# may-/joeys2t

Hardware: AMD Instinct MI355X
Metric: audio frames/sec (train step, 80-mel, 15 s utt, bs32 per GPU) (higher is better)
Workload: dtype bf16; 1 GPU; configs/librispeech_100h.yaml ASR train step on synthetic 16 kHz waveforms; global_batch=32, frames_per_utt=1498, encoder_len=375, lengths=fixed 15 s, vocab=5000, batch_multiplier=1, parallelism=dp1, launch=hipGraph replay

## Files before the change

### include/joeys2t_hip.h

```cpp
#ifndef JOEYS2T_HIP_H
#define JOEYS2T_HIP_H

#include <stdint.h>

#ifdef __cplusplus
extern "C" {
#endif

typedef void* js2t_stream;

enum { JS2T_F32 = 0, JS2T_BF16 = 1, JS2T_FP8_E4M3 = 2  };
enum { JS2T_ACT_NONE = 0, JS2T_ACT_RELU = 1, JS2T_ACT_GELU = 2, JS2T_ACT_SWISH = 3, JS2T_ACT_TANH = 4, JS2T_ACT_HARDSWISH = 5 };
enum { JS2T_OK = 0, JS2T_ERR_INVALID = -1, JS2T_ERR_LAUNCH = -2, JS2T_ERR_UNSUPPORTED = -3 };

int js2t_abi_version(void);
const char* js2t_last_error(void);

typedef struct js2t_gemm_desc {
  int32_t M, N, K;
  int32_t batch, batch_inner;
  int32_t dtype_ab, dtype_c;
  int32_t trans_a, trans_b;
  const void* A; int64_t lda, a_stride_o, a_stride_i;
  const void* B; int64_t ldb, b_stride_o, b_stride_i;
// ... 26 lines not shown
  float* c8_state;
  const float* c8_mul;
  float* c8_scale_out;
  float* fp8_state;
  const void* dot_src;
  int64_t ld_dot;
  float* dot_partial;
  float* sumsq_partial;
} js2t_gemm_desc;

int js2t_gemm(const js2t_gemm_desc* d, js2t_stream stream);
#define JS2T_GEMM_GROUP_MAX 32
int js2t_gemm_grouped(const js2t_gemm_desc* d, int32_t count, const void* const* A, const void* const* B, void* const* C,
                      float* const* a_rowsum, js2t_stream stream);
int64_t js2t_gemm_grouped_blocks(int32_t M, int32_t N, int32_t count);
void js2t_gemm_force_regstage(int on);
void js2t_gemm_force_w256(int on);
void js2t_gemm_p192_mode(int mode);
void js2t_gemm_wg256_mode(int mode);
void js2t_gemm_p192_ring(int nst);
void js2t_gemm_panel_mode(int mode);


int js2t_axpby(const void* x, float a, const void* y, float b, void* out, int64_t n, int dt, js2t_stream stream);

int js2t_cast(const void* src, int src_dt, void* dst, int dst_dt, int64_t n, js2t_stream stream);

int js2t_fold_ln_weights(const int64_t* table, int32_t n_entries, int32_t max_rows, js2t_stream stream);

int js2t_absmax(const void* x, int dt, int64_t n, float* out, js2t_stream stream);
// ... 261 lines not shown
```

### joeys2t_amd/_lib.py

```python
import ctypes as C
import os
import re
from pathlib import Path

PKG_DIR = Path(__file__).resolve().parent
LIB_PATH = Path(os.environ.get("JS2T_LIB", PKG_DIR / "libjoeys2t_hip.so"))
HEADER_PATH = PKG_DIR.parent / "include" / "joeys2t_hip.h"

F32, BF16 = 0, 1
ACT_CODES = {None: 0, "none": 0, "relu": 1, "gelu": 2, "swish": 3, "tanh": 4, "hardswish": 5}


class Js2tError(RuntimeError):
    pass


_CTYPES = {
    "int": C.c_int, "int32_t": C.c_int32, "uint32_t": C.c_uint32, "int64_t": C.c_int64, "uint64_t": C.c_uint64,
    "float": C.c_float, "double": C.c_double, "js2t_stream": C.c_void_p, "js2t_ctx": C.c_void_p,
}


def _ctype(spelling: str, decl: str, ret: bool = False):
    t = " ".join(spelling.replace("*", " * ").split())
# ... 28 lines not shown
        raise Js2tError(f"{HEADER_PATH.name}: could not parse the declaration of {sorted(missed)}")
    return structs, functions


if not HEADER_PATH.exists():
    raise Js2tError(f"{HEADER_PATH} is missing: the Python binding reads every struct and signature from it")
STRUCTS, FUNCTIONS = parse_header(HEADER_PATH.read_text())


class GemmDesc(C.Structure):
    _fields_ = STRUCTS["js2t_gemm_desc"]


class AttnDesc(C.Structure):
    _fields_ = STRUCTS["js2t_attn_desc"]


def declared_symbols():
    return sorted(FUNCTIONS)


_lib = None


def lib():
    global _lib
    if _lib is None:
        if not LIB_PATH.exists():
            raise Js2tError(
                f"{LIB_PATH} is missing: the HIP extension has not been built "
# ... 66 lines not shown
```

### joeys2t_amd/csrc/gemm.hip

```cpp
#include "gemm_shared.hpp"
#include <type_traits>

namespace {

bool g_force_regstage = false;
bool g_force_w256 = false;

__device__ __forceinline__ bool a_elem_offset(const js2t_gemm_desc& d, int slow, int fast, int64_t& off) {
  if (!d.conv) {
    off = (int64_t)slow * d.lda + fast;
    return true;
  }
  const int b = slow / d.conv_tout, t = slow - b * d.conv_tout;
  const int kw = fast / d.conv_c;
  const int tin = t * d.conv_stride - d.conv_pad + kw;
  off = ((int64_t)b * d.conv_tin + (t * d.conv_stride - d.conv_pad)) * d.conv_c + fast;
  return tin >= 0 && tin < d.conv_tin;
}

__device__ __forceinline__ void gemm_epilogue4(const js2t_gemm_desc& d, int z, int64_t c_boff, int m, int n,
                                               f32x4_t acc, float alpha) {
  if (m >= d.M || n >= d.N) return;
  const int nv = min(4, d.N - n);
  float v[4];
// ... 2223 lines not shown
          const int m = tm0 + 16 * (w + 4 * i) + 4 * g + e;
          if (m < M) __builtin_amdgcn_global_atomic_fadd_f32((gfloat*)grp.rowsum[mem] + m, racc[i][e]);
        }
    }
  }
  P192_T(6);
  asm volatile("s_waitcnt vmcnt(0)" ::: "memory");
#ifdef JS2T_P192_PROF
  if (blockIdx.x == 0 && t == 0)
    for (int i = 0; i < 8; ++i) g_p192_prof[i] = prof_[i];
#endif
}

constexpr int WG_IMG = 16384, WG_STAGE = 3 * WG_IMG, WG_NST = 3, WG_LDS = WG_NST * WG_STAGE, WG_PER = 12;

template <bool RS, bool SPLITK>
__global__ __launch_bounds__(768, 1) void gemm_bf16_wg256_kernel(js2t_gemm_desc d, GemmGroup grp, int tiles_m, int tiles_n, int split_k) {
  extern __shared__ __attribute__((aligned(16))) unsigned char smem[];
  const int t = threadIdx.x, lane = t & 63;
  const int w = __builtin_amdgcn_readfirstlane(t >> 6);
  const int tiles = tiles_m * tiles_n;
  const int lid = xcd_remap(blockIdx.x, gridDim.x);
  const int vm = lid / tiles, tile = lid - vm * tiles;
  const int mem = SPLITK ? vm / split_k : vm, slice = SPLITK ? vm - mem * split_k : 0;
  const int m0 = (tile / tiles_n) * 256, n0 = (tile % tiles_n) * 128;
  const int K = d.K, nk_all = (K + 63) >> 6;
  const int per = SPLITK ? (nk_all + split_k - 1) / split_k : nk_all;
  const int kt0 = slice * per;
  const int nk = min(per, nk_all - kt0);
  float ss = 0.f;

  if (w >= 8) {
    const int l = w - 8;
    const int64_t lda = d.lda, ldb = d.ldb;
    const uint16_t* zsrc = (const uint16_t*)&g_zero16;
    const uint16_t* src[12];
    int krow[4];
    {
      const uint16_t* Ab = (const uint16_t*)grp.A[mem];
      const uint16_t* Bb = (const uint16_t*)grp.B[mem];
#pragma unroll
      for (int q = 0; q < 4; ++q) {
        const int p = (l * 4 + q) * 64 + lane, kr = p >> 4, col = (((p & 15) ^ (tr_g(kr) << 1)) << 3);
        krow[q] = kr;
        src[q] = Ab + (int64_t)kr * lda + m0 + col;
        src[4 + q] = Ab + (int64_t)kr * lda + m0 + 128 + col;
        src[8 + q] = Bb + (int64_t)kr * ldb + n0 + col;
      }
    }
    auto issue_stage = [&](int st, int slot) {
      const int k0 = st < nk ? (kt0 + st) << 6 : 0;
      const int64_t ka = (int64_t)k0 * lda, kb = (int64_t)k0 * ldb;
      const int klim = K - k0;
      unsigned char* stp = smem + slot * WG_STAGE + l * 4096;
#pragma unroll
      for (int q = 0; q < 12; ++q) {
        const uint16_t* sp = src[q] + (q < 8 ? ka : kb);
        if (klim < 64) {
          if (krow[q & 3] >= klim) sp = zsrc;
        }
        lds_dma16(sp, stp + (q >> 2) * WG_IMG + (q & 3) * 1024);
      }
    };
    issue_stage(0, 0);
    issue_stage(1, 1);
    asm volatile("s_waitcnt vmcnt(%0)" ::"n"(WG_PER) : "memory");
    __builtin_amdgcn_s_barrier();
    asm volatile("" ::: "memory");
    issue_stage(2, 2);
    int cslot = 0;
#ifdef JS2T_P192_PROF
    unsigned long long prof_[8] = {0, 0, 0, 0, 0, 0, 0, 0}, last_ = __builtin_readcyclecounter();
#endif
    for (int s = 0; s < nk; ++s) {
// ... 10 lines not shown
#ifdef JS2T_P192_PROF
    if (blockIdx.x == 0 && t == 512)
      for (int i = 4; i < 8; ++i) g_p192_prof[i] = prof_[i];
#endif
  } else {
    const int wm = w >> 1, wn = w & 1;
    const int a_img = (wm >> 1) * WG_IMG, a_sub = (wm & 1) * 64, b_sub = wn * 64;
    bf16x8_t fm0[4], fn0[4], fm1[4], fn1[4];
    f32x4_t acc[4][4], racc[4];
#pragma unroll
    for (int i = 0; i < 4; ++i) {
      racc[i] = f32x4_t{0.f, 0.f, 0.f, 0.f};
#pragma unroll
      for (int j = 0; j < 4; ++j) acc[i][j] = f32x4_t{0.f, 0.f, 0.f, 0.f};
    }
    const bool do_rs = RS && n0 == 0 && wn == 0 && grp.rowsum[mem] != nullptr;
    typedef __attribute__((ext_vector_type(8))) short s16x8_ones_t;
    const bf16x8_t ones = __builtin_bit_cast(bf16x8_t, s16x8_ones_t{0x3f80, 0x3f80, 0x3f80, 0x3f80, 0x3f80, 0x3f80, 0x3f80, 0x3f80});

    __builtin_amdgcn_s_barrier();
    asm volatile("" ::: "memory");
#pragma unroll
    for (int i = 0; i < 4; ++i) {
      fm0[i] = frag_load2<true>(smem + a_img, a_sub + 16 * i, 0, lane);
      fn0[i] = frag_load2<true>(smem + 2 * WG_IMG, b_sub + 16 * i, 0, lane);
    }
    int cslot = 0;
#ifdef JS2T_P192_PROF
    unsigned long long prof_[8] = {0, 0, 0, 0, 0, 0, 0, 0}, last_ = __builtin_readcyclecounter();
#endif
    for (int s = 0; s < nk; ++s) {
// ... 43 lines not shown
        for (int i = 0; i < 4; ++i) racc[i] = __builtin_amdgcn_mfma_f32_16x16x32_bf16(ones, fm1[i], racc[i], 0, 0, 0);
      }
      __builtin_amdgcn_sched_barrier(0);
      P192_T(3);
      cslot = nslot;
    }
#ifdef JS2T_P192_PROF
    if (blockIdx.x == 0 && t == 0)
      for (int i = 0; i < 4; ++i) g_p192_prof[i] = prof_[i];
#endif

    if (RS && do_rs && (lane >> 4) == 0) {
      typedef __attribute__((address_space(1))) float gfloat;
#pragma unroll
      for (int i = 0; i < 4; ++i)
        __builtin_amdgcn_global_atomic_fadd_f32((gfloat*)grp.rowsum[mem] + m0 + wm * 64 + 16 * i + lane, racc[i][0]);
    }
    if constexpr (SPLITK) {
      asm volatile("s_waitcnt lgkmcnt(0)" ::: "memory");
      __syncthreads();
      float* Cs = (float*)smem;
#pragma unroll
      for (int i = 0; i < 4; ++i)
#pragma unroll
        for (int j = 0; j < 4; ++j) {
          const int ml = wm * 64 + 16 * i + (lane & 15), n4 = wn * 16 + 4 * j + (lane >> 4);
          *(f32x4_t*)(Cs + ml * 128 + ((n4 ^ (ml & 7)) << 2)) = acc[i][j];
        }
    } else {
    const float alpha = d.alpha * (d.alpha_dev ? *d.alpha_dev : 1.f), beta = d.beta;
    float* Cb = (float*)grp.C[mem] + (int64_t)(m0 + wm * 64 + (lane & 15)) * d.ldc + n0 + wn * 64 + 4 * (lane >> 4);
#pragma unroll
    for (int i = 0; i < 4; ++i) {
      float* crow = Cb + (int64_t)(16 * i) * d.ldc;
      float4 old[4];
      if (beta != 0.f) {
#pragma unroll
        for (int j = 0; j < 4; ++j) old[j] = *(const float4*)(crow + 16 * j);
      }
#pragma unroll
      for (int j = 0; j < 4; ++j) {
        float4 v = make_float4(acc[i][j][0] * alpha, acc[i][j][1] * alpha, acc[i][j][2] * alpha, acc[i][j][3] * alpha);
        if (beta != 0.f) v.x += beta * old[j].x, v.y += beta * old[j].y, v.z += beta * old[j].z, v.w += beta * old[j].w;
        *(float4*)(crow + 16 * j) = v;
        ss = fmaf(v.x, v.x, fmaf(v.y, v.y, fmaf(v.z, v.z, fmaf(v.w, v.w, ss))));
      }
    }
    }
  }
  if constexpr (SPLITK) {
    if (w >= 8) __syncthreads();
    __syncthreads();
    const float alpha = d.alpha * (d.alpha_dev ? *d.alpha_dev : 1.f);
    const float* Cs = (const float*)smem;
    typedef __attribute__((address_space(1))) float gfloat;
    gfloat* cg = (gfloat*)grp.C[mem] + (int64_t)m0 * d.ldc + n0;
    for (int idx = w; idx < 512; idx += 12) {
      const int ml = idx >> 1, nl = (idx & 1) * 64 + lane;
      const float v = Cs[ml * 128 + ((((nl >> 2) ^ (ml & 7)) << 2) | (nl & 3))];
      __builtin_amdgcn_global_atomic_fadd_f32(cg + (int64_t)ml * d.ldc + nl, v * alpha);
    }
    return;
  }
  if (d.sumsq_partial) {
    ss = block_sum(ss, (float*)smem);
    if (t == 0) d.sumsq_partial[2 * blockIdx.x] = ss, d.sumsq_partial[2 * blockIdx.x + 1] = 0.f;
  }
}

#define g_p192_mode js2t_ctx_value(JS2T_CTX_GEMM_P192_MODE)
inline bool p192_eligible(const js2t_gemm_desc& d) {
  if (g_p192_mode == 0) return false;
  if (d.trans_a || d.trans_b || d.conv || d.split_k > 1 || d.batch != 1 || d.dtype_c != JS2T_BF16) return false;
  if ((d.N & 7) || d.N < 128 || (d.K & 7) || d.K < 192 || d.M < 1) return false;
  if (d.preact || d.beta != 0.f || !(d.act == JS2T_ACT_NONE || d.act == JS2T_ACT_RELU) || (d.residual && d.gate)) return false;
  if (!epilogue_rows_aligned(d)) return false;
  if (g_p192_mode < 0 && (int64_t)cdiv(d.M, P_BM) * (d.N >> 7) < 200) return false;
  return true;
}
#define g_p192_ring js2t_ctx_value(JS2T_CTX_GEMM_P192_RING)
enum P192Form { P192_LOADER_CONSUMER, P192_RING2, P192_RING3 };
inline P192Form p192_form(int tiles, int n_cu, int ring, bool stats_dot, bool fp8, bool c8, bool scaled) {
// ... 202 lines not shown
      else
        rc = a_rowsum ? launch_grouped_wg256<true, false>(d, grp, n, (hipStream_t)stream) : launch_grouped_wg256<false, false>(d, grp, n, (hipStream_t)stream);
    } else if (!d.sumsq_partial && p192t_eligible(d, n)) {
      rc = a_rowsum ? launch_grouped_p192t<true>(d, grp, n, (hipStream_t)stream) : launch_grouped_p192t<false>(d, grp, n, (hipStream_t)stream);
    } else {
      rc = d.split_k > 1 ? launch_grouped_tt<true>(d, grp, n, (hipStream_t)stream) : launch_grouped_tt<false>(d, grp, n, (hipStream_t)stream);
    }
    if (rc != JS2T_OK) return rc;
    if (d.sumsq_partial) d.sumsq_partial += (int64_t)cdiv(d.M, 128) * cdiv(d.N, F_BN) * n;
  }
  return JS2T_OK;
}

extern "C" int64_t js2t_gemm_grouped_blocks(int32_t M, int32_t N, int32_t count) {
  return (int64_t)cdiv(M, 128) * cdiv(N, F_BN) * count;
}

extern "C" int js2t_gemm(const js2t_gemm_desc* dp, js2t_stream stream) {
  JS2T_CHECK(dp != nullptr, "gemm: null descriptor");
  js2t_gemm_desc d = *dp;
  JS2T_CHECK(!d.sumsq_partial, "gemm: sumsq_partial is taken by js2t_gemm_grouped only");
  hipStream_t s = (hipStream_t)stream;
  JS2T_CHECK(d.M >= 0 && d.N >= 0 && d.K >= 0 && d.batch >= 0, "gemm: negative size");
  if (d.M == 0 || d.N == 0 || d.batch == 0) return JS2T_OK;
  JS2T_CHECK(d.A && d.B && (d.C || (d.c8 && d.dtype_ab == JS2T_FP8_E4M3)), "gemm: null operand");
  JS2T_CHECK(!d.c8 || (d.dtype_ab == JS2T_FP8_E4M3 && d.c8_state && d.ldc8 >= d.N && (d.ldc8 & 7) == 0 && aligned(d.c8, 8) &&
                       aligned(d.c8_state)),
             "gemm: c8 (e4m3 second output) needs e4m3 operands, c8_state (16-byte aligned) and 8-byte aligned rows");
  JS2T_CHECK(d.batch_inner >= 1, "gemm: batch_inner must be >= 1");
  JS2T_CHECK(d.dtype_ab == JS2T_F32 || d.dtype_ab == JS2T_BF16 || d.dtype_ab == JS2T_FP8_E4M3, "gemm: bad dtype_ab");
// ... 71 lines not shown
```

### joeys2t_amd/ops.py

```python
import ctypes as C
import math
from typing import Optional, Sequence

import torch

from joeys2t_amd._lib import ACT_CODES, BF16, F32, AttnDesc, GemmDesc, Js2tError, check, lib

FP8 = 2
_DT = {torch.float32: F32, torch.bfloat16: BF16, torch.float8_e4m3fn: FP8}


def dt_code(t_or_dtype) -> int:
    dtype = t_or_dtype.dtype if torch.is_tensor(t_or_dtype) else t_or_dtype
    try:
        return _DT[dtype]
    except KeyError:
        raise Js2tError(f"unsupported dtype {dtype}: the HIP path computes in float32 or bfloat16") from None


def _dev(*tensors):
    for t in tensors:
        if t is not None and not t.is_cuda:
            raise Js2tError(
                "joeys2t_amd ops run on the GPU through libjoeys2t_hip.so only; got a CPU tensor "
# ... 190 lines not shown
    pa, pb, pc = arr(*[t.data_ptr() for t in As]), arr(*[t.data_ptr() for t in Bs]), arr(*[t.data_ptr() for t in Cs])
    pr = None if a_rowsums is None else arr(*[t.data_ptr() for t in a_rowsums])
    if GEMM_TIMER is not None:
        GEMM_TIMER.wrap(f"js2t_gemm_grouped<split_k {'>' if d.split_k > 1 else '='} 1> (gemm_bf16_wg256_kernel | gemm_bf16_dma_grouped_kernel)",
                        2.0 * d.M * d.N * d.K * n,
                        lambda: check(lib().js2t_gemm_grouped(C.byref(d), n, pa, pb, pc, pr, _stream()), "js2t_gemm_grouped"),
                        nbytes=n * (2 * (d.M * d.K + d.N * d.K) + Cs[0].element_size() * d.M * d.N * (2 if d.beta else 1)))
    else:
        check(lib().js2t_gemm_grouped(C.byref(d), n, pa, pb, pc, pr, _stream()), "js2t_gemm_grouped")


def grouped_blocks(M: int, N: int, count: int) -> int:
    return lib().js2t_gemm_grouped_blocks(M, N, count)


def cast(src: torch.Tensor, dtype: torch.dtype, out: Optional[torch.Tensor] = None) -> torch.Tensor:
    _dev(src, out)
    src = src.contiguous()
    if out is None:
        out = torch.empty(src.shape, dtype=dtype, device=src.device)
    check(lib().js2t_cast(_p(src), dt_code(src), _p(out), dt_code(out), src.numel(), _stream()), "js2t_cast")
    return out


def axpby(x, a: float, y=None, b: float = 0.0):
    _dev(x, y)
    out = torch.empty_like(x)
    check(lib().js2t_axpby(_p(x), a, _p(y), b, _p(out), x.numel(), dt_code(x), _stream()), "js2t_axpby")
    return out

# ... 838 lines not shown
```

### joeys2t_amd/runtime.py

```python
from typing import Dict, List, Optional, Sequence, Tuple

import torch
from torch import nn

from joeys2t_amd import ops

_ALIGN = 64


class ParamStore:

    def __init__(self, module: nn.Module, device: torch.device):
        self.device = torch.device(device)
        group_of: Dict[int, List[nn.Parameter]] = {}
        for m in module.modules():
            fg = getattr(m, "fuse_groups", None)
            if fg is None:
                continue
            for grp in fg():
                grp = [p for p in grp if p is not None]
                if any(id(p) in group_of for p in grp):
                    continue
                for p in grp:
                    group_of[id(p)] = grp
# ... 207 lines not shown
            if self.flat_lp is None:
                self.refresh()
            base = self.flat_lp
        out = base[offs[0]:offs[0] + n].view(rows, *params[0].shape[1:])
        self._cache[key] = out
        return out


class LnFold:
    __slots__ = ("w", "bias")

    def __init__(self, w, bias):
        self.w, self.bias = w, bias


class WgradQueue:

    def __init__(self, flush_every: Optional[int] = None):
        self.groups = {}
        self.pending = 0
        self.flush_every = flush_every
        self.after_flush = []
        self.cand = None
        self.kept = None
        self.first = False
        self.collector = None
        self.grad_base = None
        self._written = []

    def add(self, dz2d: torch.Tensor, x2d: torch.Tensor, dw_out: torch.Tensor, db_out: Optional[torch.Tensor]):
        N, K, M = dz2d.shape[1], x2d.shape[1], dz2d.shape[0]
        key = (N, K, M, dz2d.stride(0), x2d.stride(0), db_out is not None)
        self.groups.setdefault(key, []).append((dz2d, x2d, dw_out, db_out))
        self.pending += 1
        if self.flush_every is not None and self.pending >= self.flush_every:
            self.flush()

    def flush(self, on_group_done=None):
        self.run(self.take(), on_group_done)
        cbs, self.after_flush = self.after_flush, []
        for cb in cbs:
            cb()

# ... 2 lines not shown
        return (lo, lo + t.numel())

    def take(self, final: bool = True):
        from joeys2t_amd.functional import wgrad_split
        classes: Dict[tuple, list] = {}
        for key, items in self.groups.items():
            classes.setdefault((key[0], key[1], key[5]), []).append((key, items))
        plan = []
        for ck, members in sorted(classes.items(), key=lambda kv: -kv[0][0] * kv[0][1] * sum(len(it) for _, it in kv[1])):
            plan.extend(members)
        self.groups = {}
        self.pending = 0
        cand, out, written = self.cand, [], []
        active = cand is not None and self.grad_base is not None and self.flush_every is None
        seen: Dict[int, int] = {}
        if active:
            for _, items in plan:
                for it in items:
                    seen[it[2].data_ptr()] = seen.get(it[2].data_ptr(), 0) + 1
        for key, items in plan:
            mode = 0
            if active:
                N, K, M = key[:3]
                spans = [self._span(it[2]) for it in items]
                solo = all(seen[it[2].data_ptr()] == 1 and it[2].is_contiguous() and it[2].dtype == torch.float32 for it in items)
                unsplit = wgrad_split(N, K, M, count=len(items)) == 1 and wgrad_split(N, K, 1 << 30, count=len(items)) == 1
                if solo and unsplit and all(cand.contains(*s) for s in spans):
                    if self.first:
                        mode |= 1
                        written.extend(spans)
                    if self.collector is not None and K % 128 == 0:
                        mode |= 2
            out.append((key + (mode, self.collector if mode & 2 else None), items))
        if active and self.first:
            written = self._written + written
            self._written = [] if final else written
            if final:
                for lo, hi in self.kept.minus(written):
                    self.grad_base[lo:hi].zero_()
                    self.kept.remove(lo, hi)
            for lo, hi in written:
                if not self.kept.contains(lo, hi):
                    self.kept.add(lo, hi)
        return out

    @staticmethod
    def run(plan, on_group_done=None):
        from joeys2t_amd.functional import wgrad_split
        for key, items in plan:
            N, K, M, lda, ldb, has_db = key[:6]
            mode, collector = (key[6], key[7]) if len(key) > 6 else (0, None)
            n = len(items)
            sk = wgrad_split(N, K, M, count=n)
            part = None
            if mode & 2:
                lo = [(it[2].data_ptr() - collector.grad.data_ptr()) // 4 for it in items]
                part = collector.segment(ops.grouped_blocks(N, K, n), [(a, a + it[2].numel()) for a, it in zip(lo, items)])
            ops.gemm_grouped([it[0] for it in items], [it[1] for it in items], [it[2] for it in items], M=N, N=K, K=M, lda=lda,
                             ldb=ldb, ldc=K, split_k=sk, beta=0.0 if (sk > 1 or mode & 1) else 1.0,
                             a_rowsums=[it[3] for it in items] if has_db else None, sumsq_partial=part)
            if on_group_done is not None:
                on_group_done(items)


class RangeSet:

    def __init__(self, ranges=()):
        self.r: List[Tuple[int, int]] = []
        for lo, hi in sorted(ranges):
            if self.r and lo <= self.r[-1][1]:
                self.r[-1] = (self.r[-1][0], max(hi, self.r[-1][1]))
            elif hi > lo:
                self.r.append((lo, hi))
        self.version = 0

    def contains(self, lo: int, hi: int) -> bool:
        return any(a <= lo and hi <= b for a, b in self.r)
# ... 134 lines not shown
```

### joeys2t_amd/training.py

```python
import os
from typing import Dict, Optional

import torch

from joeys2t_amd import functional, ops
from joeys2t_amd.batch import Batch
from joeys2t_amd.builders import FlatAdamW, WarmupInverseSquareRootScheduler
from joeys2t_amd.helpers_for_ddp import FlatGradReducer, use_ddp
from joeys2t_amd.model import Model
from joeys2t_amd.runtime import WgradQueue


EARLY_EXCHANGE = os.environ.get("JS2T_EARLY_EXCHANGE", "1") != "0"


class TrainStep:
    def __init__(self, model: Model, *, learning_rate: float = 2.0e-3, adam_betas=(0.9, 0.98), weight_decay: float = 0.0,
                 clip_grad_norm: Optional[float] = 10.0, scheduling: Optional[str] = "warmupinversesquareroot",
                 learning_rate_warmup: int = 10000, learning_rate_min: float = 1.0e-6, normalization: str = "batch",
                 batch_multiplier: int = 1, n_gpu: int = 1, n_buckets: int = 4, sync_every_backward: bool = False,
                 defer_wgrads: bool = True, overlap_ctc: bool = False, comm_dtype: Optional[torch.dtype] = None, comm=None,
                 deterministic: bool = False):
        self.model = model
        from joeys2t_amd._lib import Context
# ... 31 lines not shown
                if isinstance(m, torch.nn.Linear) and uses.get(id(m.weight), 0) == 1 and m.weight.requires_grad and id(m.weight) in self.store.offsets:
                    lo = self.store.offsets[id(m.weight)]
                    spans.append((lo, lo + m.weight.numel()))
            q.cand = RangeSet(spans)
            q.kept = self.optimizer.keep = RangeSet()
            q.grad_base = self.store.flat_grad
        self.reducer = None
        if use_ddp():
            if comm is None and os.environ.get("JS2T_COMM", "") == "cabi":
                comm = "cabi"
            if comm == "cabi":
                from joeys2t_amd.comm import Communicator
                comm = Communicator.from_process_group(self.store.device)
            self.reducer = FlatGradReducer(self.store, n_buckets=n_buckets, ranges=self.store.type_ranges if defer_wgrads else None,
                                           comm_dtype=comm_dtype, comm=comm)
        self._late_leaves = [p for n, p in model.named_parameters() if n.startswith(("decoder.", "trg_embed.")) and p.requires_grad]
        self.rt.on_grads_ready = self.reducer.params_ready if (self.reducer is not None and self.rt.wgrad_queue is None) else None
        self.stats = torch.zeros(6, dtype=torch.float64, device=self.store.device)
        self._grad_seeds: Dict[float, torch.Tensor] = {}
        self.external_lr = False

    def exchange_and_flush(self, plan=None):
        q = self.rt.wgrad_queue
        with self.ctx:
            if plan is None:
                plan = q.take() if q is not None else []
            if self.reducer is None:
                WgradQueue.run(plan)
                return
            self.reducer.exchange_begin(plan)
# ... 143 lines not shown
```

Baseline: 4.322 million frames/s.

## Merge deferred weight-gradient GEMMs of mixed shapes into one tiled launch

Adds a mixed-shape wgrad GEMM path. The wg256 tile body is factored into a device function with row-tail masking, and a new kernel reads per-tile member, class and shape tables from a workspace. The deferred weight-gradient queue groups all eligible unsplit fp32 wgrads across shapes into a single launch. Tiles are load-balanced across lists and interleaved by XCD, and the tile tables are cached. The goal is to cut per-group launch overhead and tail underutilisation. The cost is host-side table building, an extra table-upload kernel, and tail-masking checks inside the tile; it is disabled under DDP.

```diff
diff --git a/include/joeys2t_hip.h b/include/joeys2t_hip.h
--- a/include/joeys2t_hip.h
+++ b/include/joeys2t_hip.h
@@ -64,6 +64,24 @@
 int js2t_gemm_grouped(const js2t_gemm_desc* d, int32_t count, const void* const* A, const void* const* B, void* const* C,
                       float* const* a_rowsum, js2t_stream stream);
 int64_t js2t_gemm_grouped_blocks(int32_t M, int32_t N, int32_t count);
+typedef struct js2t_wgrad_member {
+  const void* A;
+  const void* B;
+  void* C;
+  float* rowsum;
+  int32_t rows, cols, K;
+  int32_t sumsq_slot;
+  int64_t lda, ldb, ldc;
+  float beta;
+  int32_t reserved;
+} js2t_wgrad_member;
+typedef struct js2t_wgrad_tile {
+  int32_t member, row_tile, col_tile;
+  int32_t sumsq_slot;
+} js2t_wgrad_tile;
+int64_t js2t_gemm_wgrad_mixed_workspace(int32_t n_members, int32_t n_tiles);
+int js2t_gemm_wgrad_mixed(const js2t_wgrad_member* members, int32_t n_members, const js2t_wgrad_tile* tiles, int32_t n_tiles,
+                          float alpha, float* sumsq_partial, void* workspace, int64_t workspace_bytes, js2t_stream stream);
 void js2t_gemm_force_regstage(int on);
 void js2t_gemm_force_w256(int on);
 void js2t_gemm_p192_mode(int mode);
diff --git a/joeys2t_amd/_lib.py b/joeys2t_amd/_lib.py
--- a/joeys2t_amd/_lib.py
+++ b/joeys2t_amd/_lib.py
@@ -66,6 +66,14 @@
 
 class AttnDesc(C.Structure):
     _fields_ = STRUCTS["js2t_attn_desc"]
+
+
+class WgradMember(C.Structure):
+    _fields_ = STRUCTS["js2t_wgrad_member"]
+
+
+class WgradTile(C.Structure):
+    _fields_ = STRUCTS["js2t_wgrad_tile"]
 
 
 def declared_symbols():
diff --git a/joeys2t_amd/csrc/gemm.hip b/joeys2t_amd/csrc/gemm.hip
--- a/joeys2t_amd/csrc/gemm.hip
+++ b/joeys2t_amd/csrc/gemm.hip
@@ -1,5 +1,8 @@
 #include "gemm_shared.hpp"
+#include <algorithm>
+#include <cstring>
 #include <type_traits>
+#include <vector>
 
 namespace {
 
@@ -2261,31 +2264,35 @@
 
 constexpr int WG_IMG = 16384, WG_STAGE = 3 * WG_IMG, WG_NST = 3, WG_LDS = WG_NST * WG_STAGE, WG_PER = 12;
 
-template <bool RS, bool SPLITK>
-__global__ __launch_bounds__(768, 1) void gemm_bf16_wg256_kernel(js2t_gemm_desc d, GemmGroup grp, int tiles_m, int tiles_n, int split_k) {
-  extern __shared__ __attribute__((aligned(16))) unsigned char smem[];
+struct WgTile {
+  const void* A;
+  const void* B;
+  void* C;
+  float* rowsum;
+  float* sumsq;
+  const float* alpha_dev;
+  int m0, n0, K, kt0, nk;
+  int rows;
+  int64_t lda, ldb, ldc;
+  float alpha, beta;
+};
+template <bool RS, bool SPLITK, bool TAIL = false>
+__device__ __forceinline__ void wg256_tile(const WgTile& tl, unsigned char* smem) {
   const int t = threadIdx.x, lane = t & 63;
   const int w = __builtin_amdgcn_readfirstlane(t >> 6);
-  const int tiles = tiles_m * tiles_n;
-  const int lid = xcd_remap(blockIdx.x, gridDim.x);
-  const int vm = lid / tiles, tile = lid - vm * tiles;
-  const int mem = SPLITK ? vm / split_k : vm, slice = SPLITK ? vm - mem * split_k : 0;
-  const int m0 = (tile / tiles_n) * 256, n0 = (tile % tiles_n) * 128;
-  const int K = d.K, nk_all = (K + 63) >> 6;
-  const int per = SPLITK ? (nk_all + split_k - 1) / split_k : nk_all;
-  const int kt0 = slice * per;
-  const int nk = min(per, nk_all - kt0);
+  const int m0 = tl.m0, n0 = tl.n0, K = tl.K, kt0 = tl.kt0, nk = tl.nk;
+  const bool row_tail = TAIL && m0 + 256 > tl.rows;
   float ss = 0.f;
 
   if (w >= 8) {
     const int l = w - 8;
-    const int64_t lda = d.lda, ldb = d.ldb;
+    const int64_t lda = tl.lda, ldb = tl.ldb;
     const uint16_t* zsrc = (const uint16_t*)&g_zero16;
     const uint16_t* src[12];
     int krow[4];
     {
-      const uint16_t* Ab = (const uint16_t*)grp.A[mem];
-      const uint16_t* Bb = (const uint16_t*)grp.B[mem];
+      const uint16_t* Ab = (const uint16_t*)tl.A;
+      const uint16_t* Bb = (const uint16_t*)tl.B;
 #pragma unroll
       for (int q = 0; q < 4; ++q) {
         const int p = (l * 4 + q) * 64 + lane, kr = p >> 4, col = (((p & 15) ^ (tr_g(kr) << 1)) << 3);
@@ -2295,6 +2302,14 @@
         src[8 + q] = Bb + (int64_t)kr * ldb + n0 + col;
       }
     }
+    unsigned dead = 0;
+    if (row_tail) {
+#pragma unroll
+      for (int q = 0; q < 4; ++q) {
+        const int p = (l * 4 + q) * 64 + lane, col = (((p & 15) ^ (tr_g(p >> 4) << 1)) << 3);
+        dead |= (m0 + col >= tl.rows ? 1u : 0u) << q | (m0 + 128 + col >= tl.rows ? 1u : 0u) << (4 + q);
+      }
+    }
     auto issue_stage = [&](int st, int slot) {
       const int k0 = st < nk ? (kt0 + st) << 6 : 0;
       const int64_t ka = (int64_t)k0 * lda, kb = (int64_t)k0 * ldb;
@@ -2305,6 +2320,9 @@
         const uint16_t* sp = src[q] + (q < 8 ? ka : kb);
         if (klim < 64) {
           if (krow[q & 3] >= klim) sp = zsrc;
+        }
+        if (TAIL && row_tail && q < 8) {
+          if (dead >> q & 1) sp = zsrc;
         }
         lds_dma16(sp, stp + (q >> 2) * WG_IMG + (q & 3) * 1024);
       }
@@ -2345,7 +2363,7 @@
 #pragma unroll
       for (int j = 0; j < 4; ++j) acc[i][j] = f32x4_t{0.f, 0.f, 0.f, 0.f};
     }
-    const bool do_rs = RS && n0 == 0 && wn == 0 && grp.rowsum[mem] != nullptr;
+    const bool do_rs = RS && n0 == 0 && wn == 0 && tl.rowsum != nullptr;
     typedef __attribute__((ext_vector_type(8))) short s16x8_ones_t;
     const bf16x8_t ones = __builtin_bit_cast(bf16x8_t, s16x8_ones_t{0x3f80, 0x3f80, 0x3f80, 0x3f80, 0x3f80, 0x3f80, 0x3f80, 0x3f80});
 
@@ -2419,7 +2437,8 @@
       typedef __attribute__((address_space(1))) float gfloat;
 #pragma unroll
       for (int i = 0; i < 4; ++i)
-        __builtin_amdgcn_global_atomic_fadd_f32((gfloat*)grp.rowsum[mem] + m0 + wm * 64 + 16 * i + lane, racc[i][0]);
+        if (!TAIL || m0 + wm * 64 + 16 * i + lane < tl.rows)
+          __builtin_amdgcn_global_atomic_fadd_f32((gfloat*)tl.rowsum + m0 + wm * 64 + 16 * i + lane, racc[i][0]);
     }
     if constexpr (SPLITK) {
       asm volatile("s_waitcnt lgkmcnt(0)" ::: "memory");
@@ -2433,11 +2452,12 @@
           *(f32x4_t*)(Cs + ml * 128 + ((n4 ^ (ml & 7)) << 2)) = acc[i][j];
         }
     } else {
-    const float alpha = d.alpha * (d.alpha_dev ? *d.alpha_dev : 1.f), beta = d.beta;
-    float* Cb = (float*)grp.C[mem] + (int64_t)(m0 + wm * 64 + (lane & 15)) * d.ldc + n0 + wn * 64 + 4 * (lane >> 4);
+    const float alpha = tl.alpha * (tl.alpha_dev ? *tl.alpha_dev : 1.f), beta = tl.beta;
+    float* Cb = (float*)tl.C + (int64_t)(m0 + wm * 64 + (lane & 15)) * tl.ldc + n0 + wn * 64 + 4 * (lane >> 4);
 #pragma unroll
     for (int i = 0; i < 4; ++i) {
-      float* crow = Cb + (int64_t)(16 * i) * d.ldc;
+      if (TAIL && m0 + wm * 64 + 16 * i + (lane & 15) >= tl.rows) continue;
+      float* crow = Cb + (int64_t)(16 * i) * tl.ldc;
       float4 old[4];
       if (beta != 0.f) {
 #pragma unroll
@@ -2456,21 +2476,42 @@
   if constexpr (SPLITK) {
     if (w >= 8) __syncthreads();
     __syncthreads();
-    const float alpha = d.alpha * (d.alpha_dev ? *d.alpha_dev : 1.f);
+    const float alpha = tl.alpha * (tl.alpha_dev ? *tl.alpha_dev : 1.f);
     const float* Cs = (const float*)smem;
     typedef __attribute__((address_space(1))) float gfloat;
-    gfloat* cg = (gfloat*)grp.C[mem] + (int64_t)m0 * d.ldc + n0;
+    gfloat* cg = (gfloat*)tl.C + (int64_t)m0 * tl.ldc + n0;
     for (int idx = w; idx < 512; idx += 12) {
       const int ml = idx >> 1, nl = (idx & 1) * 64 + lane;
       const float v = Cs[ml * 128 + ((((nl >> 2) ^ (ml & 7)) << 2) | (nl & 3))];
-      __builtin_amdgcn_global_atomic_fadd_f32(cg + (int64_t)ml * d.ldc + nl, v * alpha);
+      __builtin_amdgcn_global_atomic_fadd_f32(cg + (int64_t)ml * tl.ldc + nl, v * alpha);
     }
     return;
   }
-  if (d.sumsq_partial) {
+  if (tl.sumsq) {
     ss = block_sum(ss, (float*)smem);
-    if (t == 0) d.sumsq_partial[2 * blockIdx.x] = ss, d.sumsq_partial[2 * blockIdx.x + 1] = 0.f;
-  }
+    if (t == 0) tl.sumsq[0] = ss, tl.sumsq[1] = 0.f;
+  }
+}
+
+template <bool RS, bool SPLITK>
+__global__ __launch_bounds__(768, 1) void gemm_bf16_wg256_kernel(js2t_gemm_desc d, GemmGroup grp, int tiles_m, int tiles_n, int split_k) {
+  extern __shared__ __attribute__((aligned(16))) unsigned char smem[];
+  const int tiles = tiles_m * tiles_n;
+  const int lid = xcd_remap(blockIdx.x, gridDim.x);
+  const int vm = lid / tiles, tile = lid - vm * tiles;
+  const int mem = SPLITK ? vm / split_k : vm, slice = SPLITK ? vm - mem * split_k : 0;
+  const int nk_all = (d.K + 63) >> 6;
+  const int per = SPLITK ? (nk_all + split_k - 1) / split_k : nk_all;
+  WgTile tl;
+  tl.A = grp.A[mem], tl.B = grp.B[mem], tl.C = grp.C[mem], tl.rowsum = grp.rowsum[mem];
+  tl.sumsq = d.sumsq_partial ? d.sumsq_partial + 2 * blockIdx.x : nullptr;
+  tl.alpha_dev = d.alpha_dev;
+  tl.m0 = (tile / tiles_n) * 256, tl.n0 = (tile % tiles_n) * 128, tl.K = d.K, tl.rows = d.M;
+  tl.kt0 = slice * per;
+  tl.nk = min(per, nk_all - tl.kt0);
+  tl.lda = d.lda, tl.ldb = d.ldb, tl.ldc = d.ldc;
+  tl.alpha = d.alpha, tl.beta = d.beta;
+  wg256_tile<RS, SPLITK>(tl, smem);
 }
 
 #define g_p192_mode js2t_ctx_value(JS2T_CTX_GEMM_P192_MODE)
@@ -2703,6 +2744,161 @@
 
 extern "C" int64_t js2t_gemm_grouped_blocks(int32_t M, int32_t N, int32_t count) {
   return (int64_t)cdiv(M, 128) * cdiv(N, F_BN) * count;
+}
+
+constexpr int WG_CLS_WORDS = 6, WG_MEM_WORDS = 10, WG_TILE_WORDS = 3, WG_RUN_WORDS = 5, WG_RUN_STRIDE = 8, WG_PAYLOAD_WORDS = 896;
+namespace {
+struct WgPayload {
+  uint32_t w[WG_PAYLOAD_WORDS];
+};
+__global__ __launch_bounds__(256) void wgrad_tables_kernel(WgPayload p, int n_raw, uint32_t* raw_dst, int n_runs, uint32_t* tiles_dst) {
+  const int t = blockIdx.x * 256 + threadIdx.x, nt = gridDim.x * 256;
+  for (int i = t; i < n_raw; i += nt) raw_dst[i] = p.w[i];
+  for (int r = t >> 4; r < n_runs; r += nt >> 4) {
+    const uint32_t* rw = p.w + n_raw + WG_RUN_WORDS * r;
+    const uint32_t w0 = rw[0], first = rw[1], pos = rw[2];
+    const int slot0 = (int)rw[3], sstep = (int)rw[4];
+    const uint32_t member = w0 & 0xffffu, len = (w0 >> 16) + 1;
+    for (uint32_t j = t & 15; j < len; j += 16) {
+      uint32_t* e = tiles_dst + WG_TILE_WORDS * (size_t)(pos + WG_RUN_STRIDE * j);
+      e[0] = member, e[1] = first + j, e[2] = (uint32_t)(slot0 < 0 ? -1 : slot0 + sstep * (int)j);
+    }
+  }
+}
+
+__device__ __forceinline__ uint32_t wg_word(const uint32_t* p) { return __builtin_amdgcn_readfirstlane(*p); }
+__device__ __forceinline__ void* wg_ptr(const uint32_t* p) { return (void*)(uintptr_t)((uint64_t)wg_word(p) | ((uint64_t)wg_word(p + 1) << 32)); }
+
+template <bool RS>
+__global__ __launch_bounds__(768, 1) void gemm_bf16_wg256_mixed_kernel(const uint32_t* __restrict__ classes, const uint32_t* __restrict__ members,
+                                                                       const uint32_t* __restrict__ tiles, float* sumsq_partial, float alpha) {
+  extern __shared__ __attribute__((aligned(16))) unsigned char smem[];
+  const uint32_t* te = tiles + WG_TILE_WORDS * (size_t)blockIdx.x;
+  const int tile = (int)wg_word(te + 1);
+  const uint32_t* me = members + WG_MEM_WORDS * (size_t)wg_word(te);
+  const uint32_t* ce = classes + WG_CLS_WORDS * (size_t)wg_word(me + 8);
+  const int tiles_n = (int)wg_word(ce + 1) >> 7, slot = (int)wg_word(te + 2);
+  WgTile tl;
+  tl.A = wg_ptr(me), tl.B = wg_ptr(me + 2), tl.C = wg_ptr(me + 4), tl.rowsum = (float*)wg_ptr(me + 6);
+  tl.sumsq = slot >= 0 ? sumsq_partial + slot : nullptr;
+  tl.alpha_dev = nullptr;
+  tl.m0 = (tile / tiles_n) * 256, tl.n0 = (tile % tiles_n) * 128, tl.K = (int)wg_word(ce + 2), tl.rows = (int)wg_word(ce);
+  tl.kt0 = 0, tl.nk = (tl.K + 63) >> 6;
+  tl.lda = (int)wg_word(ce + 3), tl.ldb = (int)wg_word(ce + 4), tl.ldc = (int)wg_word(ce + 5);
+  tl.alpha = alpha, tl.beta = __uint_as_float(wg_word(me + 9));
+  wg256_tile<RS, false, true>(tl, smem);
+}
+}
+
+extern "C" int64_t js2t_gemm_wgrad_mixed_workspace(int32_t n_members, int32_t n_tiles) {
+  if (n_members < 0 || n_tiles < 0) return 0;
+  return 4 * ((int64_t)(WG_CLS_WORDS + WG_MEM_WORDS) * n_members + WG_TILE_WORDS * (int64_t)n_tiles);
+}
+
+extern "C" int js2t_gemm_wgrad_mixed(const js2t_wgrad_member* mem, int32_t n_members, const js2t_wgrad_tile* tiles, int32_t n_tiles,
+                                     float alpha, float* sumsq_partial, void* workspace, int64_t workspace_bytes, js2t_stream stream) {
+  JS2T_CHECK(n_members >= 0 && n_tiles >= 0, "gemm_wgrad_mixed: bad arguments");
+  if (n_members == 0 || n_tiles == 0) {
+    JS2T_CHECK(n_members == 0 && n_tiles == 0, "gemm_wgrad_mixed: every tile of every member must be listed exactly once");
+    return JS2T_OK;
+  }
+  JS2T_CHECK(mem && tiles && n_members <= 65536, "gemm_wgrad_mixed: null tables, or more than 65536 members");
+  JS2T_CHECK(workspace && aligned(workspace) && workspace_bytes >= js2t_gemm_wgrad_mixed_workspace(n_members, n_tiles),
+             "gemm_wgrad_mixed: workspace must be 16-byte aligned and hold js2t_gemm_wgrad_mixed_workspace(members, tiles) bytes");
+  std::vector<uint32_t> raw;
+  raw.reserve((size_t)(WG_CLS_WORDS + WG_MEM_WORDS) * n_members);
+  std::vector<uint32_t> cls_of(n_members);
+  std::vector<int64_t> first_tile(n_members + 1, 0);
+  bool any_rs = false;
+  for (int i = 0; i < n_members; ++i) {
+    const js2t_wgrad_member& m = mem[i];
+    JS2T_CHECK(m.A && m.B && m.C && aligned(m.A) && aligned(m.B) && aligned(m.C), "gemm_wgrad_mixed: operands must be non-null, 16-byte aligned");
+    JS2T_CHECK(m.rows > 0 && m.cols > 0 && (m.rows & 7) == 0 && (m.cols & 127) == 0 && m.K >= 192,
+               "gemm_wgrad_mixed: rows %% 8 == 0, cols %% 128 == 0, K >= 192 (member %d: %d x %d over %d)", i, m.rows, m.cols, m.K);
+    JS2T_CHECK(m.lda >= m.rows && m.ldb >= m.cols && m.ldc >= m.cols && (m.lda & 7) == 0 && (m.ldb & 7) == 0 && (m.ldc & 3) == 0 &&
+                   m.lda <= INT32_MAX && m.ldb <= INT32_MAX && m.ldc <= INT32_MAX,
+               "gemm_wgrad_mixed: lda, ldb multiples of 8 and ldc of 4, no smaller than the rows they stride over");
+    JS2T_CHECK(m.sumsq_slot >= -1 && (m.sumsq_slot < 0 || sumsq_partial), "gemm_wgrad_mixed: sumsq_slot without sumsq_partial");
+    const uint32_t c[WG_CLS_WORDS] = {(uint32_t)m.rows, (uint32_t)m.cols, (uint32_t)m.K, (uint32_t)m.lda, (uint32_t)m.ldb, (uint32_t)m.ldc};
+    size_t k = 0;
+    for (; k < raw.size(); k += WG_CLS_WORDS)
+      if (std::equal(c, c + WG_CLS_WORDS, raw.begin() + k)) break;
+    if (k == raw.size()) raw.insert(raw.end(), c, c + WG_CLS_WORDS);
+    cls_of[i] = (uint32_t)(k / WG_CLS_WORDS);
+    first_tile[i + 1] = first_tile[i] + (int64_t)cdiv(m.rows, 256) * (m.cols >> 7);
+    any_rs = any_rs || m.rowsum != nullptr;
+  }
+  const size_t n_cls_words = raw.size();
+  for (int i = 0; i < n_members; ++i) {
+    const js2t_wgrad_member& m = mem[i];
+    const uint64_t p[4] = {(uint64_t)(uintptr_t)m.A, (uint64_t)(uintptr_t)m.B, (uint64_t)(uintptr_t)m.C, (uint64_t)(uintptr_t)m.rowsum};
+    for (int q = 0; q < 4; ++q) raw.push_back((uint32_t)p[q]), raw.push_back((uint32_t)(p[q] >> 32));
+    uint32_t beta_bits;
+    memcpy(&beta_bits, &m.beta, 4);
+    raw.push_back(cls_of[i]), raw.push_back(beta_bits);
+  }
+  JS2T_CHECK(first_tile[n_members] == n_tiles, "gemm_wgrad_mixed: every tile of every member must be listed exactly once");
+  std::vector<uint32_t> num(n_tiles);
+  std::vector<int32_t> slot(n_tiles);
+  std::vector<uint8_t> seen(n_tiles, 0);
+  for (int b = 0; b < n_tiles; ++b) {
+    const js2t_wgrad_tile& tt = tiles[b];
+    JS2T_CHECK(tt.member >= 0 && tt.member < n_members, "gemm_wgrad_mixed: tile %d names member %d", b, tt.member);
+    const js2t_wgrad_member& m = mem[tt.member];
+    JS2T_CHECK(tt.row_tile >= 0 && tt.row_tile < cdiv(m.rows, 256) && tt.col_tile >= 0 && tt.col_tile < (m.cols >> 7),
+               "gemm_wgrad_mixed: tile %d lies outside its member", b);
+    num[b] = (uint32_t)(tt.row_tile * (m.cols >> 7) + tt.col_tile);
+    JS2T_CHECK(tt.sumsq_slot >= -1 && (tt.sumsq_slot < 0 || sumsq_partial), "gemm_wgrad_mixed: tile %d: sumsq_slot without sumsq_partial", b);
+    slot[b] = tt.sumsq_slot >= 0 ? tt.sumsq_slot : (m.sumsq_slot >= 0 ? m.sumsq_slot + 2 * (int32_t)num[b] : -1);
+    uint8_t& s = seen[first_tile[tt.member] + num[b]];
+    JS2T_CHECK(!s, "gemm_wgrad_mixed: every tile of every member must be listed exactly once");
+    s = 1;
+  }
+  std::vector<uint32_t> runs;
+  for (int x = 0; x < WG_RUN_STRIDE && x < n_tiles; ++x)
+    for (int b = x; b < n_tiles;) {
+      int len = 1;
+      const int nb = b + WG_RUN_STRIDE;
+      const int sstep = (nb < n_tiles && slot[b] >= 0 && slot[nb] >= 0) ? slot[nb] - slot[b] : 0;
+      while (len < 65536 && b + WG_RUN_STRIDE * len < n_tiles && tiles[b + WG_RUN_STRIDE * len].member == tiles[b].member &&
+             num[b + WG_RUN_STRIDE * len] == num[b] + len &&
+             slot[b + WG_RUN_STRIDE * len] == (slot[b] < 0 ? -1 : slot[b] + sstep * len))
+        ++len;
+      runs.push_back((uint32_t)tiles[b].member | ((uint32_t)(len - 1) << 16)), runs.push_back(num[b]), runs.push_back((uint32_t)b);
+      runs.push_back((uint32_t)slot[b]), runs.push_back((uint32_t)sstep);
+      b += WG_RUN_STRIDE * len;
+    }
+  uint32_t* ws = (uint32_t*)workspace;
+  uint32_t* cls_dev = ws;
+  uint32_t* mem_dev = ws + n_cls_words;
+  uint32_t* tiles_dev = ws + raw.size();
+  hipStream_t s = (hipStream_t)stream;
+  const size_t n_runs = runs.size() / WG_RUN_WORDS;
+  size_t raw_at = 0, run_at = 0;
+  while (raw_at < raw.size() || run_at < n_runs) {
+    WgPayload p;
+    const size_t n_raw = std::min<size_t>(raw.size() - raw_at, WG_PAYLOAD_WORDS);
+    std::copy(raw.begin() + raw_at, raw.begin() + raw_at + n_raw, p.w);
+    uint32_t* raw_dst = ws + raw_at;
+    size_t nr = 0;
+    if (raw_at + n_raw == raw.size()) {
+      nr = std::min<size_t>(n_runs - run_at, (WG_PAYLOAD_WORDS - n_raw) / WG_RUN_WORDS);
+      std::copy(runs.begin() + WG_RUN_WORDS * run_at, runs.begin() + WG_RUN_WORDS * (run_at + nr), p.w + n_raw);
+    }
+    const int grid = (int)std::min<size_t>(8, cdiv((int)std::max<size_t>(n_raw, 16 * nr), 256));
+    hipLaunchKernelGGL(wgrad_tables_kernel, dim3(grid), dim3(256), 0, s, p, (int)n_raw, raw_dst, (int)nr, tiles_dev);
+    JS2T_LAUNCH_CHECK();
+    raw_at += n_raw, run_at += nr;
+  }
+  if (any_rs) {
+    JS2T_LDS_ONCE((gemm_bf16_wg256_mixed_kernel<true>), WG_LDS);
+    hipLaunchKernelGGL((gemm_bf16_wg256_mixed_kernel<true>), dim3(n_tiles), dim3(768), WG_LDS, s, cls_dev, mem_dev, tiles_dev, sumsq_partial, alpha);
+  } else {
+    JS2T_LDS_ONCE((gemm_bf16_wg256_mixed_kernel<false>), WG_LDS);
+    hipLaunchKernelGGL((gemm_bf16_wg256_mixed_kernel<false>), dim3(n_tiles), dim3(768), WG_LDS, s, cls_dev, mem_dev, tiles_dev, sumsq_partial, alpha);
+  }
+  JS2T_LAUNCH_CHECK();
+  return JS2T_OK;
 }
 
 extern "C" int js2t_gemm(const js2t_gemm_desc* dp, js2t_stream stream) {
diff --git a/joeys2t_amd/ops.py b/joeys2t_amd/ops.py
--- a/joeys2t_amd/ops.py
+++ b/joeys2t_amd/ops.py
@@ -4,7 +4,7 @@
 
 import torch
 
-from joeys2t_amd._lib import ACT_CODES, BF16, F32, AttnDesc, GemmDesc, Js2tError, check, lib
+from joeys2t_amd._lib import ACT_CODES, BF16, F32, AttnDesc, GemmDesc, Js2tError, WgradMember, WgradTile, check, lib
 
 FP8 = 2
 _DT = {torch.float32: F32, torch.bfloat16: BF16, torch.float8_e4m3fn: FP8}
@@ -228,6 +228,58 @@
     return lib().js2t_gemm_grouped_blocks(M, N, count)
 
 
+def wgrad_tiles(tiles):
+    arr = (WgradTile * len(tiles))()
+    for e, t in zip(arr, tiles):
+        e.member, e.row_tile, e.col_tile = t[:3]
+        e.sumsq_slot = t[3] if len(t) > 3 else -1
+    return arr
+
+
+def wgrad_mixed_slots(rows: int, cols: int) -> int:
+    return 2 * ((rows + 255) // 256) * (cols // 128)
+
+
+def gemm_wgrad_mixed(members, tiles, *, alpha=1.0, sumsq_partial=None, workspace=None):
+    n = len(members)
+    if n == 0:
+        return
+    if not isinstance(tiles, C.Array):
+        tiles = wgrad_tiles(tiles)
+    _dev(sumsq_partial, workspace, *(t for m in members for t in m[:4]))
+    arr = (WgradMember * n)()
+    for e, (a, b, c, rs, beta, slot) in zip(arr, members):
+        if a.dtype != torch.bfloat16 or b.dtype != torch.bfloat16 or c.dtype != torch.float32 or a.shape[0] != b.shape[0]:
+            raise Js2tError("gemm_wgrad_mixed: bf16 [tokens, rows] / [tokens, cols] operands and f32 outputs required")
+        if a.stride(1) != 1 or b.stride(1) != 1 or c.stride(1) != 1 or c.shape != (a.shape[1], b.shape[1]):
+            raise Js2tError("gemm_wgrad_mixed: rows of the operands must be contiguous, dW is [rows, cols]")
+        if rs is not None and (rs.dtype != torch.float32 or rs.numel() < a.shape[1] or not rs.is_contiguous()):
+            raise Js2tError("gemm_wgrad_mixed: db must be a contiguous f32 [rows]")
+        e.A, e.B, e.C, e.rowsum = a.data_ptr(), b.data_ptr(), c.data_ptr(), None if rs is None else rs.data_ptr()
+        e.rows, e.cols, e.K, e.sumsq_slot = a.shape[1], b.shape[1], a.shape[0], int(slot)
+        e.lda, e.ldb, e.ldc, e.beta = a.stride(0), b.stride(0), c.stride(0), float(beta)
+    if sumsq_partial is not None and (sumsq_partial.dtype != torch.float32 or not sumsq_partial.is_contiguous()):
+        raise Js2tError("gemm_wgrad_mixed: sumsq_partial must be contiguous f32")
+    for e in arr:
+        if e.sumsq_slot >= 0 and (sumsq_partial is None or e.sumsq_slot + wgrad_mixed_slots(e.rows, e.cols) > sumsq_partial.numel()):
+            raise Js2tError("gemm_wgrad_mixed: sumsq_slot outside sumsq_partial")
+    top = max((t.sumsq_slot for t in tiles), default=-1)
+    if top >= 0 and (sumsq_partial is None or top + 2 > sumsq_partial.numel()):
+        raise Js2tError("gemm_wgrad_mixed: a tile's sumsq_slot outside sumsq_partial")
+    need = lib().js2t_gemm_wgrad_mixed_workspace(n, len(tiles))
+    if workspace is None:
+        workspace = torch.empty((need, ), dtype=torch.uint8, device=members[0][2].device)
+    elif workspace.dtype != torch.uint8 or workspace.numel() < need or not workspace.is_contiguous():
+        raise Js2tError(f"gemm_wgrad_mixed: workspace must be a contiguous uint8 tensor of {need} bytes")
+    call = lambda: check(lib().js2t_gemm_wgrad_mixed(arr, n, tiles, len(tiles), float(alpha), _p(sumsq_partial), _p(workspace),
+                                                     workspace.numel(), _stream()), "js2t_gemm_wgrad_mixed")
+    if GEMM_TIMER is not None:
+        GEMM_TIMER.wrap("js2t_gemm_wgrad_mixed (gemm_bf16_wg256_mixed_kernel)", sum(2.0 * e.rows * e.cols * e.K for e in arr), call,
+                        nbytes=sum(2 * e.K * (e.rows + e.cols) + 4 * e.rows * e.cols * (2 if e.beta else 1) for e in arr))
+    else:
+        call()
+
+
 def cast(src: torch.Tensor, dtype: torch.dtype, out: Optional[torch.Tensor] = None) -> torch.Tensor:
     _dev(src, out)
     src = src.contiguous()
diff --git a/joeys2t_amd/runtime.py b/joeys2t_amd/runtime.py
--- a/joeys2t_amd/runtime.py
+++ b/joeys2t_amd/runtime.py
@@ -1,3 +1,4 @@
+import os
 from typing import Dict, List, Optional, Sequence, Tuple
 
 import torch
@@ -245,6 +246,56 @@
         self.w, self.bias = w, bias
 
 
+WGRAD_LISTS = 8
+
+
+def wgrad_merge_shape(rows: int, cols: int, tokens: int) -> bool:
+    return rows > 0 and rows % 8 == 0 and cols > 0 and cols % 128 == 0 and tokens >= 192
+
+
+def wgrad_tile_lists(shapes, lists: int = WGRAD_LISTS):
+    classes: Dict[tuple, list] = {}
+    for i, sh in enumerate(shapes):
+        classes.setdefault(tuple(sh), []).append(i)
+    out = [[] for _ in range(lists)]
+    load = [0] * lists
+    for (rows, cols, tokens), members in sorted(classes.items(), key=lambda kv: (-((kv[0][2] + 63) // 64), kv[1][0])):
+        tm, tn, cost = (rows + 255) // 256, cols // 128, (tokens + 63) // 64
+        row = [(m, r, c) for m in members for r in range(tm) for c in range(tn)]
+        q, rest = divmod(len(row), lists)
+        longer = set(sorted(range(lists), key=lambda x: (load[x], x))[:rest])
+        pos = 0
+        for x in range(lists):
+            n = q + (x in longer)
+            out[x].extend(row[pos:pos + n])
+            load[x] += n * cost
+            pos += n
+    return out
+
+
+def wgrad_tile_order(shapes, lists: int = WGRAD_LISTS):
+    per = wgrad_tile_lists(shapes, lists)
+    return [l[i] for i in range(max(map(len, per), default=0)) for l in per if i < len(l)]
+
+
+_TILE_ARRAYS: Dict[tuple, object] = {}
+
+
+def grouped_sumsq_slots(tiles_per_member: int, count: int, group_max: int = 32):
+    out, base = [], 0
+    for m0 in range(0, count, group_max):
+        n = min(group_max, count - m0)
+        G = tiles_per_member * n
+        q, r = G >> 3, G & 7
+        at = [0] * G
+        for b in range(G):
+            xcd, idx = b & 7, b >> 3
+            at[(xcd * (q + 1) if xcd < r else r * (q + 1) + (xcd - r) * q) + idx] = base + 2 * b
+        out.extend(at[i * tiles_per_member:(i + 1) * tiles_per_member] for i in range(n))
+        base += 2 * G
+    return out
+
+
 class WgradQueue:
 
     def __init__(self, flush_every: Optional[int] = None):
@@ -258,6 +309,7 @@
         self.collector = None
         self.grad_base = None
         self._written = []
+        self.merge = int(os.environ.get("JS2T_WGRAD_MERGE", "1") or 0)
 
     def add(self, dz2d: torch.Tensor, x2d: torch.Tensor, dw_out: torch.Tensor, db_out: Optional[torch.Tensor]):
         N, K, M = dz2d.shape[1], x2d.shape[1], dz2d.shape[0]
@@ -290,24 +342,30 @@
         cand, out, written = self.cand, [], []
         active = cand is not None and self.grad_base is not None and self.flush_every is None
         seen: Dict[int, int] = {}
-        if active:
+        if active or self.merge:
             for _, items in plan:
                 for it in items:
                     seen[it[2].data_ptr()] = seen.get(it[2].data_ptr(), 0) + 1
         for key, items in plan:
             mode = 0
+            N, K, M = key[:3]
+            merged = bool(self.merge) and wgrad_merge_shape(N, K, M) and all(
+                it[2].dtype == torch.float32 and it[2].is_contiguous() and it[2].data_ptr() % 16 == 0 for it in items)
+            merged = merged and all(seen[it[2].data_ptr()] == 1 for it in items)
+            if self.merge == 1:
+                merged = merged and wgrad_split(N, K, M, count=len(items)) == 1
             if active:
-                N, K, M = key[:3]
                 spans = [self._span(it[2]) for it in items]
                 solo = all(seen[it[2].data_ptr()] == 1 and it[2].is_contiguous() and it[2].dtype == torch.float32 for it in items)
-                unsplit = wgrad_split(N, K, M, count=len(items)) == 1 and wgrad_split(N, K, 1 << 30, count=len(items)) == 1
+                unsplit = (merged and self.merge == 2) or (wgrad_split(N, K, M, count=len(items)) == 1 and
+                                                           wgrad_split(N, K, 1 << 30, count=len(items)) == 1)
                 if solo and unsplit and all(cand.contains(*s) for s in spans):
                     if self.first:
                         mode |= 1
                         written.extend(spans)
                     if self.collector is not None and K % 128 == 0:
                         mode |= 2
-            out.append((key + (mode, self.collector if mode & 2 else None), items))
+            out.append((key + (mode, self.collector if mode & 2 else None, merged), items))
         if active and self.first:
             written = self._written + written
             self._written = [] if final else written
@@ -323,20 +381,56 @@
     @staticmethod
     def run(plan, on_group_done=None):
         from joeys2t_amd.functional import wgrad_split
-        for key, items in plan:
+        parts = {}
+        for idx, (key, items) in enumerate(plan):
+            if len(key) > 6 and key[6] & 2:
+                N, K, collector = key[0], key[1], key[7]
+                as_merged = len(key) > 8 and key[8] and on_group_done is None
+                lo = [(it[2].data_ptr() - collector.grad.data_ptr()) // 4 for it in items]
+                n_entries = ops.wgrad_mixed_slots(N, K) * len(items) if as_merged else ops.grouped_blocks(N, K, len(items))
+                parts[idx] = collector.segment(n_entries, [(a, a + it[2].numel()) for a, it in zip(lo, items)])
+        if on_group_done is None:
+            WgradQueue._run_merged([(key, items, parts.get(idx)) for idx, (key, items) in enumerate(plan) if len(key) > 8 and key[8]])
+        for idx, (key, items) in enumerate(plan):
             N, K, M, lda, ldb, has_db = key[:6]
             mode, collector = (key[6], key[7]) if len(key) > 6 else (0, None)
+            merged = len(key) > 8 and key[8]
+            if merged and on_group_done is None:
+                continue
             n = len(items)
-            sk = wgrad_split(N, K, M, count=n)
-            part = None
-            if mode & 2:
-                lo = [(it[2].data_ptr() - collector.grad.data_ptr()) // 4 for it in items]
-                part = collector.segment(ops.grouped_blocks(N, K, n), [(a, a + it[2].numel()) for a, it in zip(lo, items)])
+            sk = 1 if merged else wgrad_split(N, K, M, count=n)
+            part = parts.get(idx)
             ops.gemm_grouped([it[0] for it in items], [it[1] for it in items], [it[2] for it in items], M=N, N=K, K=M, lda=lda,
                              ldb=ldb, ldc=K, split_k=sk, beta=0.0 if (sk > 1 or mode & 1) else 1.0,
                              a_rowsums=[it[3] for it in items] if has_db else None, sumsq_partial=part)
             if on_group_done is not None:
                 on_group_done(items)
+
+    @staticmethod
+    def _run_merged(plan):
+        members, shapes, slots, partial = [], [], [], None
+        for key, items, seg in plan:
+            N, K, M, has_db, mode, collector = key[0], key[1], key[2], key[5], key[6], key[7]
+            slot, per = -1, ops.wgrad_mixed_slots(N, K)
+            if seg is not None:
+                partial, slot = collector.partial, seg.storage_offset()
+            alone = slot >= 0 and N % 256 == 0 and M >= 1024 and (per // 2) * min(len(items), 32) >= 160
+            for i, it in enumerate(items):
+                members.append((it[0], it[1], it[2], it[3] if has_db else None, 0.0 if mode & 1 else 1.0, slot + i * per if slot >= 0 else -1))
+                shapes.append((N, K, M))
+            slots.append((slot, alone, len(items), per // 2))
+        if not members:
+            return
+        cache_key = (tuple(shapes), tuple(slots))
+        tiles = _TILE_ARRAYS.get(cache_key)
+        if tiles is None:
+            own = []
+            for slot, alone, n, t in slots:
+                own.extend([[slot + s for s in ms] for ms in grouped_sumsq_slots(t, n)] if alone else [None] * n)
+            order = wgrad_tile_order(shapes)
+            tiles = _TILE_ARRAYS[cache_key] = ops.wgrad_tiles(
+                [(m, r, c, -1 if own[m] is None else own[m][r * (shapes[m][1] // 128) + c]) for m, r, c in order])
+        ops.gemm_wgrad_mixed(members, tiles, sumsq_partial=partial)
 
 
 class RangeSet:
diff --git a/joeys2t_amd/training.py b/joeys2t_amd/training.py
--- a/joeys2t_amd/training.py
+++ b/joeys2t_amd/training.py
@@ -69,6 +69,8 @@
                 comm = Communicator.from_process_group(self.store.device)
             self.reducer = FlatGradReducer(self.store, n_buckets=n_buckets, ranges=self.store.type_ranges if defer_wgrads else None,
                                            comm_dtype=comm_dtype, comm=comm)
+            if q is not None:
+                q.merge = 0
         self._late_leaves = [p for n, p in model.named_parameters() if n.startswith(("decoder.", "trg_embed.")) and p.requires_grad]
         self.rt.on_grads_ready = self.reducer.params_ready if (self.reducer is not None and self.rt.wgrad_queue is None) else None
         self.stats = torch.zeros(6, dtype=torch.float64, device=self.store.device)
```

Result: no change. 4.360 million frames/s, median of 6 (+0.9%).
